# zm0612/funny_lidar_slam

Hardware: AMD Instinct MI355X
Metric: scans/sec (64-ring×1800 pts → 1e6-pt iVox map), SE(3) err vs CPU ref (higher is better)
Workload: dtype f64; 1 GPU; BASELINE configs[1]: Velodyne-64 synthetic scan (64x1800 = 115,200 pts), point-to-plane (LoamPointToPlaneIVOX semantics, YAML config_nclt.yaml) into a 1e6-pt iVox map, 1 scan per GPU per step (the same scan on every GPU); scan_points=115200, map_points=1000000, converged=True, pre_warm_matches=256

## Files before the change

### funny_lidar_slam_amd/_lib.py

```python
from __future__ import annotations

import ctypes as C
import os
import subprocess

_HERE = os.path.dirname(os.path.abspath(__file__))
LIB_PATH = os.environ.get("FLS_REG_LIB") or os.path.join(_HERE, "libfls_reg.so")
CSRC_DIR = os.path.join(_HERE, "csrc")

EXPORTED_SYMBOLS = [
    "fls_create", "fls_destroy", "fls_add_cloud_to_local_map", "fls_match", "fls_get_fitness_score",
    "fls_scan_upload", "fls_scan_upload_raw", "fls_match_resident", "fls_match_batch", "fls_map_export", "fls_map_import", "fls_map_image_bytes", "fls_map_image_export", "fls_map_image_import", "fls_get_iteration_log", "fls_get_correspondences", "fls_map_size",
    "fls_set_profiling", "fls_get_kernel_time", "fls_get_traffic_counters", "fls_get_debug_stamps", "fls_debug_fullpiv_qr6", "fls_debug_ldlt6", "fls_debug_voxel_grid", "fls_debug_voxel_grid_timed", "fls_debug_exact_sort", "fls_debug_exact_sort_marks", "fls_voxel_grid_cloud", "fls_loop_match", "fls_status_string", "fls_abi_version", "fls_abi_revision",
    "fls_device_count",
    "fls_replicas_create", "fls_replicas_refresh", "fls_replicas_match_batch", "fls_replicas_import_ms", "fls_replicas_destroy",
    "fls_features_create", "fls_features_destroy", "fls_features_project", "fls_features_extract", "fls_features_get", "fls_features_get_time",
]
HANDOFF_SYMBOLS = ["fls_preprocess_scan_device", "fls_scan_attach_preprocessed", "fls_preprocess_get_host_bytes"]
PREPROCESS_SYMBOLS = [
    "fls_preprocess_create", "fls_preprocess_destroy", "fls_preprocess_scan", "fls_preprocess_get", "fls_preprocess_get_time",
    "fls_features_project_deskew",
] + HANDOFF_SYMBOLS

FEATURES_DEVICE_SYMBOLS = ["fls_features_device_revision", "fls_features_keep_on_device", "fls_features_get_host_bytes", "fls_features_stat",
                           "fls_scan_attach_features"]
FEAT_STAT_DEVICE_GATHERS, FEAT_STAT_DEVICE_FILTERS, FEAT_STAT_FILTER_DECLINES, FEAT_STAT_LAZY_DOWNLOADS = range(4)

INGEST_SYMBOLS = ["fls_ingest_revision", "fls_ingest_default_layout", "fls_preprocess_scan_driver", "fls_features_project_driver"]

KEYFRAMES_SYMBOLS = ["fls_keyframes_revision", "fls_keyframes_create", "fls_keyframes_destroy", "fls_keyframes_add", "fls_keyframes_add_preprocessed",
                     "fls_keyframes_count", "fls_keyframes_get", "fls_keyframes_merge", "fls_keyframes_loop_match", "fls_keyframes_stat"]

LOCALMAP_SYMBOLS = ["fls_localmap_revision", "fls_localmap_create", "fls_localmap_destroy", "fls_localmap_set_global", "fls_localmap_crop",
                    "fls_localmap_split", "fls_localmap_add_tile", "fls_localmap_tiles", "fls_localmap_get_tile", "fls_localmap_load_tiles",
                    "fls_localmap_reset", "fls_localmap_get_local", "fls_add_localmap_to_local_map", "fls_localmap_stat"]

BATCH_SYMBOLS = ["fls_batch_revision", "fls_match_batch_fused", "fls_batch_stat"]

BATCH_IVOX_SYMBOLS = ["fls_batch_ivox_revision", "fls_match_batch_shared_ivox", "fls_batch_ivox_stat"]

DEBUG_LINALG_SYMBOLS = ["fls_debug_linalg_revision", "fls_debug_plane_fit_5x3", "fls_debug_svd3", "fls_debug_lu6", "fls_debug_so3", "fls_debug_wave_sum"]

DEBUG_FIT_SYMBOLS = ["fls_debug_fit_revision", "fls_debug_plane_residual", "fls_debug_line_residual", "fls_debug_icp_point_rows", "fls_debug_rank1_mfma",
                     "fls_debug_rank1_dpp", "fls_debug_rank1x3_mfma", "fls_debug_reduce_partials", "fls_debug_fanin", "fls_debug_last_system"]
DEBUG_TICKET_WORDS = 320

DEBUG_NDT_SYMBOLS = ["fls_debug_ndt_revision", "fls_debug_ndt_voxels"]

DEBUG_LOOP_SYMBOLS = ["fls_debug_loop_revision", "fls_debug_loop_ndt", "fls_debug_loop_gicp_cov", "fls_debug_loop_gicp_corr", "fls_debug_loop_gicp_fdf",
                      "fls_debug_loop_fitness"]

DEBUG_KNN_SYMBOLS = ["fls_debug_knn_revision", "fls_debug_grid_knn5", "fls_debug_grid_knn5_dual", "fls_debug_icp_knn1"]

NDT_IMAGE_SYMBOLS = ["fls_ndt_image_revision"]
NDT_IMAGE_MAGIC, NDT_IMAGE_HEADER_BYTES, NDT_IMAGE_CARRY = b"FLSNDT01", 64, 8


class NdtImageHeader(C.Structure):

    _fields_ = [("magic", C.c_char * 8), ("revision", C.c_uint32), ("carry", C.c_uint32), ("total_bytes", C.c_uint64), ("n_voxels", C.c_uint64),
                ("next_vid", C.c_int32), ("flag_first_scan", C.c_uint32), ("ndt_voxel_size_bits", C.c_uint64), ("ndt_min_points_in_voxel", C.c_int32),
                ("ndt_max_points_in_voxel", C.c_int32), ("ndt_capacity", C.c_int32), ("reserved", C.c_uint32)]


def ndt_image_layout(n: int) -> dict:
    out, o = {}, NDT_IMAGE_HEADER_BYTES
    for name, width in (("key", 8), ("num_points", 4), ("vid", 4), ("estimated", 1), ("pending", 1), ("points", NDT_IMAGE_CARRY * 24), ("mu", 24),
                        ("sigma", 72), ("info", 72)):
        out[name] = o
        o = (o + n * width + 15) & ~15
    out["total"] = o
    return out

KD_IMAGE_SYMBOLS = ["fls_kd_image_revision", "fls_replicas_match_batch_fused"]
KD_IMAGE_MAGIC, KD_IMAGE_HEADER_BYTES = b"FLSKDM01", 224


class KdImageHeader(C.Structure):

    _fields_ = [("magic", C.c_char * 8), ("revision", C.c_uint32), ("kind", C.c_uint32), ("total_bytes", C.c_uint64), ("n_maps", C.c_uint32),
                ("is_localization_mode", C.c_uint32), ("filter_size_bits", C.c_uint32 * 2), ("local_size", C.c_uint32 * 2),
                ("point_search_thres_bits", C.c_uint64), ("gate_init", C.c_uint32), ("reserved", C.c_uint32), ("gate_last_T", C.c_double * 16),
                ("n_clouds", C.c_uint64 * 2), ("n_points", C.c_uint64 * 2)]


# ... 393 lines not shown
            L.fls_debug_fanin.restype = C.c_int
            L.fls_debug_fanin.argtypes = [C.c_int, C.c_int, C.c_int, dp, u32p, u32p]
            L.fls_debug_last_system.restype = C.c_int
            L.fls_debug_last_system.argtypes = [hp, dp, dp]
        if hasattr(L, "fls_debug_ndt_revision"):
            L.fls_debug_ndt_revision.restype = C.c_int
            L.fls_debug_ndt_revision.argtypes = []
            L.fls_debug_ndt_voxels.restype = C.c_int
            L.fls_debug_ndt_voxels.argtypes = [hp, C.c_size_t, ip, ip, ip, bp, bp, dp, dp, dp, C.POINTER(C.c_size_t)]
        if hasattr(L, "fls_debug_loop_revision"):
            i64p = C.POINTER(C.c_int64)
            L.fls_debug_loop_revision.restype = C.c_int
            L.fls_debug_loop_revision.argtypes = []
            L.fls_debug_loop_ndt.restype = C.c_int
            L.fls_debug_loop_ndt.argtypes = [C.c_int, fp, C.c_int, fp, C.c_int, C.c_int, C.c_float, dp, C.c_int, dp, dp, dp, i64p, ip, ip]
            L.fls_debug_loop_gicp_cov.restype = C.c_int
            L.fls_debug_loop_gicp_cov.argtypes = [C.c_int, fp, C.c_int, C.c_int, C.c_float, C.c_double, C.c_int, dp]
            L.fls_debug_loop_gicp_corr.restype = C.c_int
            L.fls_debug_loop_gicp_corr.argtypes = [C.c_int, fp, C.c_int, fp, C.c_int, C.c_int, fp, dp, dp, dp, C.c_double, C.c_int, ip, dp]
            L.fls_debug_loop_gicp_fdf.restype = C.c_int
            L.fls_debug_loop_gicp_fdf.argtypes = [C.c_int, fp, C.c_int, fp, C.c_int, C.c_int, dp, ip, dp, C.c_int, dp]
            L.fls_debug_loop_fitness.restype = C.c_int
            L.fls_debug_loop_fitness.argtypes = [C.c_int, fp, C.c_int, fp, C.c_int, C.c_int, fp, C.c_int, dp, i64p]
        if hasattr(L, "fls_debug_knn_revision"):
            L.fls_debug_knn_revision.restype = C.c_int
            L.fls_debug_knn_revision.argtypes = []
            L.fls_debug_grid_knn5.restype = C.c_int
            L.fls_debug_grid_knn5.argtypes = [C.c_int, fp, C.c_int, fp, C.c_int, C.c_int, C.c_float, C.c_int, C.c_float, dp, C.c_int, fp, bp, fp, ip]
            L.fls_debug_grid_knn5_dual.restype = C.c_int
            L.fls_debug_grid_knn5_dual.argtypes = [C.c_int, fp, C.c_int, fp, C.c_int, C.c_float, C.c_int, C.c_float, fp, C.c_int, fp, C.c_int, C.c_float, C.c_int,
                                                   C.c_float, C.c_int, dp, C.c_int, fp, bp, fp, ip, fp, bp, fp, ip]
            L.fls_debug_icp_knn1.restype = C.c_int
            L.fls_debug_icp_knn1.argtypes = [C.c_int, fp, C.c_int, fp, C.c_int, C.c_int, C.c_float, C.c_double, dp, C.c_int, ip, bp, ip]
        if hasattr(L, "fls_ndt_image_revision"):
            L.fls_ndt_image_revision.restype = C.c_int
            L.fls_ndt_image_revision.argtypes = []
        if hasattr(L, "fls_kd_image_revision"):
            L.fls_kd_image_revision.restype = C.c_int
            L.fls_kd_image_revision.argtypes = []
            L.fls_replicas_match_batch_fused.restype = C.c_int
            L.fls_replicas_match_batch_fused.argtypes = L.fls_replicas_match_batch.argtypes
        L.fls_status_string.restype = C.c_char_p
        L.fls_status_string.argtypes = [C.c_int]
        L.fls_abi_version.restype = C.c_int
        L.fls_abi_revision.restype = C.c_int
        L.fls_device_count.restype = C.c_int
        _lib = L
    return _lib


def status_string(s: int) -> str:
    return lib().fls_status_string(int(s)).decode()


def device_count() -> int:
    return int(lib().fls_device_count())
```

### funny_lidar_slam_amd/csrc/abi_common.hpp

```cpp
#pragma once
#include <chrono>
#include "matcher_p2plane_ivox.hpp"
#include "matchers_kd.hpp"
#include "matcher_ndt.hpp"
#include "features_host.hpp"
#include "preprocess_host.hpp"
#include "loop_closure.hpp"
#include "replicas.hpp"
#include "keyframes.hpp"
#include "localmap.hpp"
#include "kernels_debug_linalg.hpp"
#include "kernels_debug_fit.hpp"
#include "../../include/fls_keyframes.h"
#include "../../include/fls_localmap.h"
#include "../../include/fls_batch.h"
#include "../../include/fls_batch_ivox.h"
#include "../../include/fls_debug_linalg.h"
#include "../../include/fls_debug_fit.h"
#include "../../include/fls_debug_ndt.h"
#include "../../include/fls_debug_loop.h"
#include "../../include/fls_debug_knn.h"
#include "../../include/fls_map_kd.h"
#include <new>
#include <type_traits>

namespace fls {

inline fls_status gfx950_device(int device_id, bool say = false) {
    int n = 0;
    hipDeviceProp_t prop;
    if (hipGetDeviceCount(&n) != hipSuccess || device_id < 0 || device_id >= n || hipGetDeviceProperties(&prop, device_id) != hipSuccess) return FLS_ERR_DEVICE;
    const char* arch = prop.gcnArchName;
    if (std::strncmp(arch, "gfx950", 6) == 0) return FLS_OK;
    if (say) std::fprintf(stderr, "[fls_reg] device %d is %s; this library is built for gfx950 only\n", device_id, arch);
    return FLS_ERR_DEVICE;
}

template <typename F>
fls_status guarded_nomem(F&& f) {
    return guarded([&]() -> fls_status {
        try {
            return f();
        } catch (const HipError& e) {
            if (e.code != hipErrorOutOfMemory) throw;
            (void)hipGetLastError();
            return FLS_ERR_NOMEM;
        }
    });
}

template <class H, class F>
fls_status on_device(H* h, F&& body) {
    return guarded([&]() -> fls_status { FLS_HIP(hipSetDevice(h->device)); return body(); });
}
// ... 63 lines not shown
```

### funny_lidar_slam_amd/csrc/abi_debug_knn.hpp

```cpp
#pragma once
#include "abi_common.hpp"

namespace {

fls_status debug_knn_device(int device_id) {
    const fls_status dev = gfx950_device(device_id);
    if (dev == FLS_OK) FLS_HIP(hipSetDevice(device_id));
    return dev;
}
inline bool debug_knn_common_ok(const float* map, int nm, const float* query, int nq, int stride, float cell, int host_grid) {
    return map && query && nm >= 0 && nq >= 0 && stride >= 3 && cell > 0.f && std::isfinite(cell) && (host_grid == 0 || host_grid == 1);
}
struct DebugKnnSide {
    LoopMatcher::DevCloud map, query;
    CellGridImage grid;
    DeviceGridBuilder builder;
    DevBuf<float4> pts;
    DevBuf<unsigned char> cnt, flag;
    DevBuf<float> kth;
    int nq = 0;
    fls_status prepare_grid(const float* m, int nm, const float* q, int n_query, int stride, float cell, int rings, bool host_grid) {
        const std::vector<PtI> mc = cloud_from(m, size_t(nm), stride), qc = cloud_from(q, size_t(n_query), stride);
        nq = n_query;
        map.upload(mc, nullptr);
// ... 2 lines not shown
        return grid.build(mc, cell, nullptr, rings, false);
    }
    void prepare_outputs() {
        pts.reserve(size_t(nq) * 5); cnt.reserve(size_t(nq)); flag.reserve(size_t(nq)); kth.reserve(size_t(nq));
        FLS_HIP(hipMemset(pts.p, 0x7b, size_t(nq) * 5 * sizeof(float4)));
        FLS_HIP(hipMemset(cnt.p, 0x7b, size_t(nq)));
        FLS_HIP(hipMemset(flag.p, 0x7b, size_t(nq)));
        FLS_HIP(hipMemset(kth.p, 0x7b, size_t(nq) * sizeof(float)));
    }
    GridKnnArgs args(float gate) { return GridKnnArgs{query.x(), query.y(), query.z(), nq, cell_dev(grid), gate, pts.p, cnt.p, kth.p, flag.p}; }
    void fetch(float* out_pts, uint8_t* out_cnt, float* out_kth, int32_t* out_has_window) {
        FLS_HIP(hipMemcpy(out_pts, pts.p, size_t(nq) * 5 * sizeof(float4), hipMemcpyDeviceToHost));
        FLS_HIP(hipMemcpy(out_cnt, cnt.p, size_t(nq), hipMemcpyDeviceToHost));
        FLS_HIP(hipMemcpy(out_kth, kth.p, size_t(nq) * sizeof(float), hipMemcpyDeviceToHost));
        *out_has_window = grid.have_window ? 1 : 0;
    }
};
inline void debug_knn_empty(int nq, float* out_pts, uint8_t* out_cnt, float* out_kth, int32_t* out_has_window) {
    const int32_t none = -1;
    for (size_t i = 0; i < size_t(nq) * 5; ++i) {
        out_pts[4 * i] = out_pts[4 * i + 1] = out_pts[4 * i + 2] = 0.f;
        std::memcpy(out_pts + 4 * i + 3, &none, sizeof(none));
    }
    for (int i = 0; i < nq; ++i) { out_cnt[i] = 0; out_kth[i] = INFINITY; }
    *out_has_window = 0;
}
inline Pose16 debug_knn_pose(const double* T16) { Pose16 T; std::memcpy(T.m, T16, sizeof(T.m)); return T; }

}

extern "C" {

int fls_debug_knn_revision(void) { return FLS_DEBUG_KNN_REVISION; }

fls_status fls_debug_grid_knn5(int device_id, const float* map, int nm, const float* query, int nq, int stride, float cell, int rings, float gate,
                               const double* T16, int host_grid, float* out_pts, uint8_t* out_cnt, float* out_kth, int32_t* out_has_window) {
    if (!debug_knn_common_ok(map, nm, query, nq, stride, cell, host_grid) || !T16 || !out_pts || !out_cnt || !out_kth || !out_has_window || (rings != 1 && rings != 2) ||
        gate != gate)
        return FLS_ERR_INVALID;
    if (nm == 0 || nq == 0) { debug_knn_empty(nq, out_pts, out_cnt, out_kth, out_has_window); return FLS_OK; }
    return guarded([&]() -> fls_status {
        fls_status rc = debug_knn_device(device_id);
        if (rc != FLS_OK) return rc;
        DebugKnnSide s;
        rc = s.prepare_grid(map, nm, query, nq, stride, cell, rings, host_grid != 0);
        if (rc != FLS_OK) return rc;
        s.prepare_outputs();
        DevBuf<GnState> st;
        st.reserve(1);
        FLS_HIP(hipMemset(st.p, 0, sizeof(GnState)));
        const GridKnnArgs a = s.args(gate);
        const dim3 knn_grid_dim(knn_grid_blocks(size_t(nq)));
        const Pose16 T0 = debug_knn_pose(T16);
        if (std::isinf(gate))
            hipLaunchKernelGGL((grid_knn_kernel<5, false, true>), knn_grid_dim, dim3(256), 0, nullptr, a.sx, a.sy, a.sz, a.n, (const GnState*)st.p, 1, T0, a.cg, gate, a.nn_pts,
                               a.nn_cnt, a.kth_d2, a.flag_to_clear);
        else
            hipLaunchKernelGGL((grid_knn_kernel<5, false>), knn_grid_dim, dim3(256), 0, nullptr, a.sx, a.sy, a.sz, a.n, (const GnState*)st.p, 1, T0, a.cg, gate, a.nn_pts,
                               a.nn_cnt, a.kth_d2, a.flag_to_clear);
        FLS_HIP(hipGetLastError());
        FLS_HIP(hipDeviceSynchronize());
        s.fetch(out_pts, out_cnt, out_kth, out_has_window);
        return FLS_OK;
    });
}

// ... 71 lines not shown
```

### funny_lidar_slam_amd/csrc/device_common.hpp

```cpp
#pragma once
#include <hip/hip_runtime.h>
#include <stdint.h>

namespace fls {

constexpr int kMaxIter = 64;
constexpr int kPartialStride = 32;
constexpr unsigned long long kEmptyKey = ~0ull;
constexpr int kKeyLimit = (1 << 20) - 2;

struct HashEntry {
    unsigned long long key;
    unsigned begin;
    unsigned count;
};
static_assert(sizeof(HashEntry) == 16, "one dwordx4 per probe");

struct DevGrid {
    const HashEntry* table;
    const float4* pts;
    unsigned mask;
    unsigned n_pts;
};

// ... 149 lines not shown
#pragma unroll
    for (int k = 0; k < NV; ++k) p[k] = a[k] = 0u;
    for (int j = threadIdx.x; j < n; j += blockDim.x) {
        const T4 e = v[j];
        const unsigned* w = reinterpret_cast<const unsigned*>(&e);
#pragma unroll
        for (int k = 0; k < NV; ++k) { a[k] += w[k]; if (j < cut) p[k] += w[k]; }
    }
    const int lane = threadIdx.x & 63, wv = threadIdx.x >> 6, nw = blockDim.x >> 6;
#pragma unroll
    for (int k = 0; k < NV; ++k) {
#pragma unroll
        for (int o = 32; o > 0; o >>= 1) { p[k] += __shfl_xor(p[k], o, 64); a[k] += __shfl_xor(a[k], o, 64); }
    }
    if (lane == 0) {
#pragma unroll
        for (int k = 0; k < NV; ++k) { wsum[wv][k] = p[k]; wsum[wv][NV + k] = a[k]; }
    }
    __syncthreads();
#pragma unroll
    for (int k = 0; k < NV; ++k) {
        unsigned sp = 0u, sa = 0u;
        for (int q = 0; q < nw; ++q) { sp += wsum[q][k]; sa += wsum[q][NV + k]; }
        pre[k] = sp; all[k] = sa;
    }
    __syncthreads();
}
#endif

struct Pose16 { double m[16]; };

struct TrafficCounters {
    unsigned long long probes, hits, cand;
};

__host__ __device__ __forceinline__ unsigned long long pack_key(int x, int y, int z) {
    return ((unsigned long long)((unsigned)x & 0x1FFFFFu) << 42) | ((unsigned long long)((unsigned)y & 0x1FFFFFu) << 21) |
           (unsigned long long)((unsigned)z & 0x1FFFFFu);
}
__host__ __device__ __forceinline__ void unpack_key(unsigned long long k, int& x, int& y, int& z) {
    x = (int)((unsigned)(k >> 42) << 11) >> 11;
    y = (int)((unsigned)((k >> 21) & 0x1FFFFFu) << 11) >> 11;
    z = (int)((unsigned)(k & 0x1FFFFFu) << 11) >> 11;
}
__host__ __device__ __forceinline__ unsigned hash_key(unsigned long long k) {
    k ^= k >> 33;
    k *= 0xff51afd7ed558ccdULL;
    k ^= k >> 33;
    k *= 0xc4ceb9fe1a85ec53ULL;
    k ^= k >> 33;
    return (unsigned)k;
}

__device__ __forceinline__ unsigned evict_merged_rank(const unsigned* __restrict__ crank, const unsigned C, const unsigned* S, const unsigned nS, const unsigned k) {
    unsigned j = 0;
    while (j < nS && j <= k && S[j] < (k - j < C ? crank[k - j] : 0xFFFFFFFFu)) ++j;
    unsigned v = 0u;
    if (j <= k && k - j < C) v = crank[k - j];
    if (j > 0u && S[j - 1] > v) v = S[j - 1];
    return v;
}

}
```

### funny_lidar_slam_amd/csrc/kernels_ivox_coop.hpp

```cpp
#pragma once
#include "kernels_p2plane.hpp"
#include "lane_group.hpp"

namespace fls {

__device__ __forceinline__ void nearby18(const int k, int& dx, int& dy, int& dz) {
    constexpr unsigned long long DX = 0x1548889561ull, DY = 0x895429495ull, DZ = 0x282956155ull;
    dx = (int)((DX >> (2 * k)) & 3ull) - 1;
    dy = (int)((DY >> (2 * k)) & 3ull) - 1;
    dz = (int)((DZ >> (2 * k)) & 3ull) - 1;
}

constexpr int nearby18_slab(const int k) {
    constexpr unsigned long long DX = 0x1548889561ull, DY = 0x895429495ull, DZ = 0x282956155ull;
    const int dx = (int)((DX >> (2 * k)) & 3ull) - 1, dy = (int)((DY >> (2 * k)) & 3ull) - 1, dz = (int)((DZ >> (2 * k)) & 3ull) - 1;
    return (dz * kBrickStored + dy) * kBrickStored + dx;
}
constexpr unsigned nearby18_slab_pack4(const int r) {
    unsigned pk = 0u;
    for (int s = 0; s < 4; ++s) {
        const int k = s + 4 * r;
        pk |= ((unsigned)(k < 19 ? nearby18_slab(k) : 0) & 0xffu) << (8 * s);
    }
    return pk;
// ... 4 lines not shown
__device__ __forceinline__ double kmin_f64(const double a, const double b) {
    double r;
    asm("v_min_f64 %0, %1, %2" : "=v"(r) : "v"(a), "v"(b));
    return r;
}
__device__ __forceinline__ double kmax_f64(const double a, const double b) {
    double r;
    asm("v_max_f64 %0, %1, %2" : "=v"(r) : "v"(a), "v"(b));
    return r;
}
__device__ __forceinline__ double make_dkey(const float d2, const unsigned slot, const bool ok) {
    return __hiloint2double((int)(ok ? __float_as_uint(d2) + kKeyBias : kKeyNoneHi), (int)slot);
}
__device__ __forceinline__ bool dkey_valid(const double k) { return (unsigned)__double2hiint(k) < kKeyValidLimit; }
__device__ __forceinline__ unsigned dkey_slot(const double k) { return (unsigned)__double2loint(k); }
__device__ __forceinline__ void top5_insert_dkey(double (&t)[5], const double key) {
    double x = kmin_f64(t[4], key);
#pragma unroll
    for (int j = 3; j >= 0; --j) {
        const double lo = kmin_f64(t[j], x), hi = kmax_f64(t[j], x);
        t[j + 1] = hi;
        x = lo;
    }
    t[0] = x;
}
template <int STEP>
__device__ __forceinline__ double dpp_min_dkey(const double v) {
    const unsigned lo = dpp_pair_u32<STEP>((unsigned)__double2loint(v));
    const unsigned hi = dpp_pair_u32<STEP>((unsigned)__double2hiint(v));
    return kmin_f64(v, __hiloint2double((int)hi, (int)lo));
}
__device__ __forceinline__ double group_min_dkey(const double v) { return dpp_min_dkey<1>(dpp_min_dkey<0>(v)); }

constexpr int kIvoxKnnQueries = 256 / 4;
#define FLS_IVOX_KNN_SMEM_PARAMS unsigned (&s_end)[kIvoxKnnQueries][24], unsigned (&s_off)[kIvoxKnnQueries][24]
#define FLS_IVOX_KNN_SMEM_DECL                                                             \
    __shared__ __attribute__((aligned(16))) unsigned s_end[kIvoxKnnQueries][24];           \
    __shared__ __attribute__((aligned(16))) unsigned s_off[kIvoxKnnQueries][24]
#define FLS_IVOX_KNN_SMEM_ARGS s_end, s_off
template <bool COUNT, bool DENSE, bool FIRST, bool GEN, class P>
__device__ __forceinline__ void
ivox_knn_body(FLS_IVOX_KNN_SMEM_PARAMS, const float* __restrict__ sx, const float* __restrict__ sy, const float* __restrict__ sz, const int n,
              const GnState* __restrict__ st, const P& T0p , const DevGrid grid, const BrickDir bd,
              const float inv_res, float4* __restrict__ nn_pts , unsigned char* __restrict__ nn_cnt,
              unsigned char* __restrict__ flag, TrafficCounters* __restrict__ tc, const int chunk,
              unsigned* __restrict__ nn_ids ,
              const int nn_prev ,
              float* __restrict__ dev_copy ) {
    const Pose16& T0 = T0p;
    constexpr int G = 4;
    constexpr int QPB = kIvoxKnnQueries;
    constexpr int R = (19 + G - 1) / G;
    const int nb = (n + QPB - 1) / QPB;
    const int xcd = blockIdx.x & 7, seq = blockIdx.x >> 3;
    const int lb = ((seq / chunk) * 8 + xcd) * chunk + (seq % chunk);
    const int sub = threadIdx.x % G;
    const int q = lb * QPB + threadIdx.x / G;
    const bool active = lb < nb && q < n;
    const int done = FIRST ? 0 : st->done;
    double T[12];
#pragma unroll
    for (int c = 0; c < 4; ++c)
#pragma unroll
        for (int r = 0; r < 3; ++r) T[c * 3 + r] = FIRST ? T0.m[c * 4 + r] : st->T[c * 4 + r];
    const int qq = active ? q : 0;
    const float px = sx[qq], py = sy[qq], pz = sz[qq];
    if (done) return;
    if (FIRST && active && sub == 0) {
        if (dev_copy) { dev_copy[q] = px; dev_copy[(size_t)n + q] = py; dev_copy[2 * (size_t)n + q] = pz; }
        flag[q] = 0;
        if (q >= nn_prev) nn_cnt[q] = 0;
    }
    const double x = px, y = py, z = pz;
    const float ptx = (float)(((T[0] * x + T[3] * y) + T[6] * z) + T[9]);
    const float pty = (float)(((T[1] * x + T[4] * y) + T[7] * z) + T[10]);
    const float ptz = (float)(((T[2] * x + T[5] * y) + T[8] * z) + T[11]);
    const float fx = roundf(ptx * inv_res), fy = roundf(pty * inv_res), fz = roundf(ptz * inv_res);
    const bool in_range = active && fabsf(fx) < (float)kKeyLimit && fabsf(fy) < (float)kKeyLimit && fabsf(fz) < (float)kKeyLimit;
    const int kx = in_range ? (int)fx : 0, ky = in_range ? (int)fy : 0, kz = in_range ? (int)fz : 0;

    const double kNone = __hiloint2double((int)kKeyNoneHi, -1);
    double t5[5] = {kNone, kNone, kNone, kNone, kNone};
    unsigned long long c_hits = 0, c_cand = 0, c_probes = 0;
    auto probe_key = [&](const int r, bool& pv) -> unsigned long long {
        const int k = sub + G * r;
        pv = in_range && k < 19;
        int ox, oy, oz;
        nearby18(k < 19 ? k : 0, ox, oy, oz);
        return pack_key(kx + ox, ky + oy, kz + oz);
    };
    auto first_load = [&](const bool pv, const unsigned long long key, unsigned& h) -> HashEntry {
        h = hash_key(key) & grid.mask;
        return pv ? grid.table[h] : HashEntry{kEmptyKey, 0u, 0u};
    };
    auto resolve = [&](const bool pv, const unsigned long long key, unsigned h, HashEntry ek, unsigned& beg, unsigned& cnt) {
        while (pv && ek.key != key && ek.key != kEmptyKey) {
            h = (h + 1) & grid.mask;
            ek = grid.table[h];
        }
        const bool hit = pv && ek.key == key;
        beg = hit ? ek.begin : 0u;
        cnt = hit ? ek.count : 0u;
        if (COUNT && pv) { c_probes++; if (hit) { c_hits++; c_cand += ek.count; } }
    };
    unsigned b0 = 0, b1 = 0, b2 = 0, b3 = 0, b4 = 0, c0 = 0, c1 = 0, c2 = 0, c3 = 0, c4 = 0;
    if (DENSE) {
        const int bx = kx >> kBrickLog, by = ky >> kBrickLog, bz = kz >> kBrickLog;
        const unsigned long long bkey = pack_key(bx, by, bz);
        unsigned h = brick_hash(bx, by, bz) & bd.mask;
        HashEntry be = bd.table[h];
        while (be.key != bkey && be.key != kEmptyKey) {
            h = (h + 1) & bd.mask;
            be = bd.table[h];
        }
        const bool have = in_range && be.key == bkey && be.begin < bd.n_cap;
        const unsigned cbase = (have ? be.begin : 0u) * kBrickStride +
                               brick_slab_index((kx & (kBrickSide - 1)) + 1, (ky & (kBrickSide - 1)) + 1, (kz & (kBrickSide - 1)) + 1);
        constexpr unsigned PK[5] = {nearby18_slab_pack4(0), nearby18_slab_pack4(1), nearby18_slab_pack4(2), nearby18_slab_pack4(3), nearby18_slab_pack4(4)};
        const unsigned sub8 = 8u * (unsigned)sub;
        auto cell = [&](const int r, const unsigned pk4, unsigned& beg, unsigned& cnt) {
            const int k = sub + G * r;
            const int off = __builtin_amdgcn_sbfe((int)pk4, sub8, 8u);
            const bool ok = have && k < 19;
            const uint2 e = bd.cells[cbase + (unsigned)off];
            beg = e.x;
            cnt = ok ? e.y : 0u;
            if (COUNT && active && k < 19) { c_probes++; if (cnt) { c_hits++; c_cand += cnt; } }
        };
        cell(0, PK[0], b0, c0);
        cell(1, PK[1], b1, c1);
        cell(2, PK[2], b2, c2);
        cell(3, PK[3], b3, c3);
        cell(4, PK[4], b4, c4);
    } else {
        bool pv0 = false, pv1 = false, pv2 = false, pv3 = false, pv4 = false;
        unsigned long long k0 = 0, k1 = 0, k2 = 0, k3 = 0, k4 = 0;
        unsigned h0 = 0, h1 = 0, h2 = 0, h3 = 0, h4 = 0;
        HashEntry e0{kEmptyKey, 0u, 0u}, e1 = e0, e2 = e0, e3 = e0, e4 = e0;
        k0 = probe_key(0, pv0); e0 = first_load(pv0, k0, h0);
        k1 = probe_key(1, pv1); e1 = first_load(pv1, k1, h1);
        k2 = probe_key(2, pv2); e2 = first_load(pv2, k2, h2);
        k3 = probe_key(3, pv3); e3 = first_load(pv3, k3, h3);
        k4 = probe_key(4, pv4); e4 = first_load(pv4, k4, h4);
        resolve(pv0, k0, h0, e0, b0, c0);
        resolve(pv1, k1, h1, e1, b1, c1);
        resolve(pv2, k2, h2, e2, b2, c2);
        resolve(pv3, k3, h3, e3, b3, c3);
        resolve(pv4, k4, h4, e4, b4, c4);
        if (COUNT && active && !in_range) {
#pragma unroll
            for (int r = 0; r < R; ++r) c_probes += sub + G * r < 19 ? 1u : 0u;
        }
    }
    auto consider = [&](const float4 p, const unsigned s, const bool ok) {
        const float dx = p.x - ptx, dy = p.y - pty, dz = p.z - ptz;
        const float d2 = dx * dx + (dy * dy + dz * dz);
        top5_insert_dkey(t5, make_dkey(d2, s, GEN ? ok && d2 < 25.0f : ok));
    };
    auto map_pt = [&](const unsigned s) -> float4 {
        if (GEN) return grid.pts[s];
        return *reinterpret_cast<const float4*>(reinterpret_cast<const char*>(grid.pts) + (s << 4));
    };
    const unsigned tot = c0 + c1 + c2 + c3 + c4;
    const int g = threadIdx.x / G;
    const unsigned nz = (c0 ? 1u : 0u) + (c1 ? 1u : 0u) + (c2 ? 1u : 0u) + (c3 ? 1u : 0u) + (c4 ? 1u : 0u);
    const unsigned packed = tot * 32u + nz;
    const unsigned t0 = (unsigned)__builtin_amdgcn_update_dpp(0, (int)packed, 0x00, 0xf, 0xf, true);
    const unsigned t1 = (unsigned)__builtin_amdgcn_update_dpp(0, (int)packed, 0x55, 0xf, 0xf, true);
    const unsigned t2 = (unsigned)__builtin_amdgcn_update_dpp(0, (int)packed, 0xAA, 0xf, 0xf, true);
    const unsigned t3 = (unsigned)__builtin_amdgcn_update_dpp(0, (int)packed, 0xFF, 0xf, 0xf, true);
    const unsigned before = (sub > 0 ? t0 : 0u) + (sub > 1 ? t1 : 0u) + (sub > 2 ? t2 : 0u), all = t0 + t1 + t2 + t3;
    const unsigned TOT = all >> 5;
    unsigned pos = before & 31u, run = before >> 5;
    {
        uint2* const rowp = reinterpret_cast<uint2*>(&s_end[g][6 * sub]);
        rowp[0] = make_uint2(~0u, ~0u); rowp[1] = make_uint2(~0u, ~0u); rowp[2] = make_uint2(~0u, ~0u);
    }
    const unsigned dmy = 20u + (unsigned)sub;
    auto put = [&](const unsigned b, const unsigned c) {
        const unsigned at = c ? pos : dmy;
        s_off[g][at] = b - run;
        run += c;
        s_end[g][at] = run;
        pos += c ? 1u : 0u;
    };
    put(b0, c0);
    put(b1, c1);
    put(b2, c2);
    put(b3, c3);
    put(b4, c4);
    s_end[g][dmy] = ~0u;
    __builtin_amdgcn_fence(__ATOMIC_RELEASE, "wavefront");
    __builtin_amdgcn_wave_barrier();
    __builtin_amdgcn_fence(__ATOMIC_ACQUIRE, "wavefront");
    const unsigned Q = (TOT + 3u) >> 2, a = sub * Q, e = a + Q < TOT ? a + Q : TOT;
    const unsigned P2 = t0 + t1, P3 = P2 + t2, A32 = a * 32u + 31u;
    unsigned ps = t0 <= A32 ? t0 : 0u;
    ps = P2 <= A32 ? P2 : ps;
    ps = P3 <= A32 ? P3 : ps;
    unsigned k = ps & 31u;
    {
        const unsigned* const w = &s_end[g][k];
        const unsigned w0 = w[0], w1 = w[1], w2 = w[2], w3 = w[3], w4 = w[4];
        k += (w0 <= a ? 1u : 0u) + (w1 <= a ? 1u : 0u) + (w2 <= a ? 1u : 0u) + (w3 <= a ? 1u : 0u) + (w4 <= a ? 1u : 0u);
    }
    for (unsigned idx = a; idx < e;) {
        const unsigned E0 = s_end[g][k], E1 = s_end[g][k + 1];
        const unsigned O0 = s_off[g][k], O1 = s_off[g][k + 1];
        const unsigned last = (E1 < e ? E1 : e) - 1;
        const unsigned i1 = idx + 1, i2 = idx + 2, i3 = idx + 3;
        const unsigned j1 = i1 < last ? i1 : last, j2 = i2 < last ? i2 : last, j3 = i3 < last ? i3 : last;
        const unsigned s0 = idx + O0;
        const unsigned s1 = j1 + (j1 < E0 ? O0 : O1);
        const unsigned s2 = j2 + (j2 < E0 ? O0 : O1);
        const unsigned s3 = j3 + (j3 < E0 ? O0 : O1);
        const float4 q0 = map_pt(s0), q1 = map_pt(s1), q2 = map_pt(s2), q3 = map_pt(s3);
        consider(q0, s0, true);
        consider(q1, s1, i1 <= last);
        consider(q2, s2, i2 <= last);
        consider(q3, s3, i3 <= last);
        idx = j3 + 1;
        k += (E0 <= idx ? 1u : 0u) + (E1 <= idx ? 1u : 0u);
    }
    const double m0 = group_min_dkey(t5[0]);
    if (dkey_valid(m0)) {
        int cnt = 0;
        unsigned sid[5] = {~0u, ~0u, ~0u, ~0u, ~0u};
#pragma unroll
        for (int j = 0; j < 5; ++j) {
            const double m = j == 0 ? m0 : group_min_dkey(t5[0]);
            const bool mv = dkey_valid(m);
            cnt += mv ? 1 : 0;
            if (mv && __double_as_longlong(t5[0]) == __double_as_longlong(m)) {
                t5[0] = t5[1]; t5[1] = t5[2]; t5[2] = t5[3]; t5[3] = t5[4]; t5[4] = kNone;
            }
            if (nn_ids) sid[j] = mv ? dkey_slot(m) : ~0u;
            else if (sub == 0 && active) {
                nn_pts[(size_t)q * 5 + j] = mv ? grid.pts[dkey_slot(m)] : make_float4(0.f, 0.f, 0.f, __int_as_float(-1));
            }
        }
        if (nn_ids) {
            if (sub == 0 && active) {
                *reinterpret_cast<uint4*>(nn_ids + (size_t)q * 8) = make_uint4(sid[0], sid[1], sid[2], sid[3]);
                nn_ids[(size_t)q * 8 + 4] = sid[4];
            }
            if (sub == 0 && active) nn_cnt[q] = (unsigned char)cnt;
        } else {
            if (sub == 0 && active) nn_cnt[q] = (unsigned char)(cnt | 0x80);
        }
    }
    if (COUNT) {
        const double p = wave_sum_u((double)c_probes), hsum = wave_sum_u((double)c_hits), c = wave_sum_u((double)c_cand);
        if ((threadIdx.x & 63) == 0) {
            atomicAdd(&tc->probes, (unsigned long long)p);
            atomicAdd(&tc->hits, (unsigned long long)hsum);
// ... 366 lines not shown
```

### funny_lidar_slam_amd/csrc/matcher_base.hpp

```cpp
#pragma once
#include "host_maps.hpp"
#include "kernels_handoff.hpp"
#include "kernels_p2plane.hpp"
#include <functional>
#include <memory>
#include <thread>
#if defined(__SSE__)
#include <xmmintrin.h>
#endif

struct fls_matcher {
    fls_kind kind;
    fls_params p{};
    int device = 0;
    hipStream_t stream = nullptr;
    fls_stats stats{};

    fls::DevBuf<fls::GnState> d_state;
    fls::PinnedBuf<fls::GnState> h_state;
    fls::DevBuf<double> d_partials_a, d_partials_b;
    fls::DevBuf<fls::TrafficCounters> d_tc;
    fls::PinnedBuf<fls::TrafficCounters> h_tc;

    bool profiling = false;
    bool count_traffic = false;
    static constexpr int kEvRing = 64;
    std::vector<hipEvent_t> ev_pool;
    hipEvent_t* ev = nullptr;
    int ev_slot = -1;
    struct PendingEv { int slot, iters; };
    std::vector<PendingEv> ev_pending;
    double prof_ms = 0.0;
    int64_t prof_launches = 0;
    uint64_t prof_point_iters = 0;
    fls::TrafficCounters last_tc{0, 0, 0};

    int log_n = 0;
    bool log_stale = false;

    fls::Mailbox* mb_host = nullptr;
    fls::Mailbox* mb_dev = nullptr;
    unsigned match_id = 0;
    bool tail_exact = false;
    unsigned launch_word() const { return fls::LaunchWord::pack(match_id, tail_exact, p.max_iterations).w; }

    virtual ~fls_matcher() {
        for (hipEvent_t e : slot_ev) if (e) (void)hipEventDestroy(e);
        for (hipEvent_t e : batch_tail_ev) if (e) (void)hipEventDestroy(e);
        if (batch_stream) { (void)hipStreamSynchronize(batch_stream); (void)hipStreamDestroy(batch_stream); }
        for (auto e : ev_pool) if (e) (void)hipEventDestroy(e);
        if (stream) { (void)hipStreamSynchronize(stream); (void)hipStreamDestroy(stream); }
        if (mb_host) (void)hipHostFree(mb_host);
    }
    virtual fls_status add_cloud(const float* c0, size_t n0, const float* c1, size_t n1, int stride) = 0;
    using HostRows = std::function<const std::vector<fls::PtI>&()>;
    virtual fls_status add_cloud_device(const fls::HandoffCloud&, const HostRows& rows, bool* took_planes) {
        *took_planes = false;
        const std::vector<fls::PtI>& r = rows();
        return add_cloud(r.empty() ? nullptr : &r[0].x, r.size(), nullptr, 0, 4);
    }
    virtual fls_status scan_upload(const float* s0, size_t n0, const float* s1, size_t n1, int stride) = 0;
    virtual fls_status scan_upload_for_match(const float* s0, size_t n0, const float* s1, size_t n1, int stride) { return scan_upload(s0, n0, s1, n1, stride); }
    virtual fls_status scan_upload_raw(const float* s0, size_t n0, const float* s1, size_t n1, int stride) { return scan_upload(s0, n0, s1, n1, stride); }
    virtual fls_status scan_attach_device(const fls::HandoffCloud&) { return FLS_ERR_STATE; }
    virtual fls_status scan_attach_features(const fls::HandoffCloud& , const fls::HandoffCloud& ) { return FLS_ERR_STATE; }
    virtual fls_status match_resident(double* T, int update_map, fls_stats* out) = 0;
    virtual fls_status fitness(float max_range, float* score) = 0;
    virtual int correspondences(int slot, int32_t* ids, uint8_t* cnt, uint8_t* valid, size_t cap) = 0;
// ... 435 lines not shown
```

### funny_lidar_slam_amd/csrc/matcher_p2plane_ivox.hpp

```cpp
#pragma once
#include "matcher_base.hpp"
#include "kernels_p2plane.hpp"
#include "kernels_knn.hpp"
#include "kernels_ivox_coop.hpp"
#include "kernels_ivox_update.hpp"
#include "ivox_map.hpp"
#include "kernels_localmap.hpp"
#include "fitness_host.hpp"
#include <thread>
#include <chrono>
#include <hip/hip_ext.h>

namespace fls {

constexpr int kIvoxXcdChunk = 8;

struct P2PlaneIvoxMatcher final : fls_matcher {
    IvoxMap map;
    const IvoxMap* borrowed = nullptr;
    const IvoxMap& read_map() const { return borrowed ? *borrowed : map; }
    bool host_timing = false;
    bool spec_pending = false;
    DevBuf<unsigned char> d_code;
    DevBuf<float4> d_pw;
// ... 523 lines not shown

    std::unique_ptr<fls_matcher> clone_for_lane() override {
        auto q = make_lane(*this);
        if (q) q->borrowed = &map;
        return q;
    }
    fls_status prepare_batch() override {
        map.refresh();
        FLS_HIP(hipStreamSynchronize(stream));
        return FLS_OK;
    }

    fls_status fitness(float max_range, float* score) override {
        if (!p.is_localization_mode) { *score = std::numeric_limits<float>::max(); return FLS_OK; }
        if (!have_fitness_grid || !have_final) return FLS_ERR_STATE;
        return fitness_score_device(*this, fitness_grid, scan, final_T, max_range, score);
    }

    int correspondences(int, int32_t* ids, uint8_t* cnt, uint8_t* valid, size_t cap) override {
        download_nn();
        const size_t n = std::min(cap, nn_n);
        h_flag.resize(nn_n);
        if (nn_n) {
            FLS_HIP(hipMemcpyAsync(h_flag.data(), d_flag.p, nn_n, hipMemcpyDeviceToHost, stream));
            FLS_HIP(hipStreamSynchronize(stream));
        }
        for (size_t i = 0; i < n; ++i) {
            cnt[i] = h_cnt[i];
            for (int j = 0; j < 5; ++j) ids[i * 5 + j] = j < h_cnt[i] ? h_nn[i * 5 + j].id : -1;
            valid[i] = h_flag[i];
        }
        return int(n);
    }
    size_t map_size(int slot) const override { return map.counter(slot); }
};

}
```

### funny_lidar_slam_amd/registration.py

```python
from __future__ import annotations

import ctypes as C
from dataclasses import dataclass, field

import numpy as np

from . import _lib
from ._lib import FlsError, Params, Stats

FloatNaN = float(np.finfo(np.float32).max)

kPointToPlane_IVOX_HIP = "PointToPlane_IVOX_HIP"
kPointToPlane_KdTree_HIP = "PointToPlane_KdTree_HIP"
kLoamFull_KdTree_HIP = "LoamFull_KdTree_HIP"
kIcpOptimized_HIP = "IcpOptimized_HIP"
kIncrementalNDT_HIP = "IncrementalNDT_HIP"


@dataclass
class PointcloudCluster:
    ordered_cloud_: np.ndarray = field(default_factory=lambda: np.zeros((0, 3), np.float32))
    planar_cloud_: np.ndarray = field(default_factory=lambda: np.zeros((0, 3), np.float32))
    corner_cloud_: np.ndarray = field(default_factory=lambda: np.zeros((0, 3), np.float32))
    raw_cloud_: np.ndarray = None
# ... 241 lines not shown
    def map_size(self, slot: int = 0) -> int:
        return int(_lib.lib().fls_map_size(self._h, slot))

    def ndt_voxels(self) -> dict:
        L = _lib.lib()
        cnt = C.c_size_t(0)
        rc = L.fls_debug_ndt_voxels(self._h, 0, None, None, None, None, None, None, None, None, C.byref(cnt))
        if rc not in (_lib.FLS_OK, _lib.FLS_ERR_NOMEM):
            raise FlsError(rc, "fls_debug_ndt_voxels")
        n = int(cnt.value)
        out = dict(keys=np.zeros((n, 3), np.int32), vid=np.zeros(n, np.int32), num_points=np.zeros(n, np.int32), estimated=np.zeros(n, np.uint8),
                   pending=np.zeros(n, np.uint8), mu=np.zeros((n, 3)), sigma=np.zeros((n, 9)), info=np.zeros((n, 9)))
        if n:
            ip, bp, dp = C.POINTER(C.c_int32), C.POINTER(C.c_uint8), C.POINTER(C.c_double)
            rc = L.fls_debug_ndt_voxels(self._h, n, out["keys"].ctypes.data_as(ip), out["vid"].ctypes.data_as(ip), out["num_points"].ctypes.data_as(ip),
                                        out["estimated"].ctypes.data_as(bp), out["pending"].ctypes.data_as(bp), out["mu"].ctypes.data_as(dp),
                                        out["sigma"].ctypes.data_as(dp), out["info"].ctypes.data_as(dp), C.byref(cnt))
            if rc != _lib.FLS_OK or int(cnt.value) != n:
                raise FlsError(rc, "fls_debug_ndt_voxels")
        return out

    def set_profiling(self, events: bool, counters: bool = False) -> None:
        _lib.lib().fls_set_profiling(self._h, (1 if events else 0) | (2 if counters else 0))

    def kernel_time(self):
        ms = C.c_double(); n = C.c_int64(); pi = C.c_uint64()
        _lib.lib().fls_get_kernel_time(self._h, C.byref(ms), C.byref(n), C.byref(pi))
        return ms.value, n.value, pi.value

    def traffic_counters(self):
        a = C.c_uint64(); b = C.c_uint64(); c = C.c_uint64()
        _lib.lib().fls_get_traffic_counters(self._h, C.byref(a), C.byref(b), C.byref(c))
        return a.value, b.value, c.value

    def close(self) -> None:
        if getattr(self, "_h", None) and self._h.value:
            _lib.lib().fls_destroy(self._h)
            self._h = C.c_void_p()

    def __del__(self):
        try:
            self.close()
        except Exception:
            pass


class LoamPointToPlaneIVOX(RegistrationInterface):

    KIND = _lib.P2PLANE_IVOX

    def __init__(self, point_to_planar_thres, position_converge_thres, rotation_converge_thres, opti_iter_num=30,
                 is_localization_mode=False, device_id=0):
        super().__init__(Params(point_to_planar_thres=point_to_planar_thres, position_converge_thres=position_converge_thres,
                                rotation_converge_thres=rotation_converge_thres, max_iterations=opti_iter_num,
                                is_localization_mode=int(is_localization_mode)), device_id)


class IcpOptimized(RegistrationInterface):

    KIND = _lib.ICP_OPTIMIZED
    K = 1

    def __init__(self, max_iterations, local_map_size, map_cloud_filter_size, source_cloud_filter_size, max_correspond_distance,
                 position_converge_thres, rotation_converge_thres, rot_thre_add_cloud, dist_thre_add_cloud,
                 is_localization_mode=False, device_id=0):
        super().__init__(Params(max_iterations=max_iterations, local_map_size=local_map_size,
# ... 189 lines not shown
```

Before: 11170 scans/s.

## Share iVox KNN candidate staging across queries in the same voxel within a wave

Adds a wave-level shared path to the dense iVox KNN. When the wave's 16 queries fall into at most three distinct voxels and their combined 19-cell neighbourhoods hold at most 256 candidates, the wave probes the cells once and stages the map points in LDS. Each query group then scans its run's staged candidates instead of probing and gathering independently. This is meant to cut redundant hash probes and global point loads for spatially coherent scans. In exchange it adds ballot, scan and barrier overhead, and it falls back to the old path when the run or capacity limits are exceeded.

```diff
diff --git a/funny_lidar_slam_amd/_lib.py b/funny_lidar_slam_amd/_lib.py
--- a/funny_lidar_slam_amd/_lib.py
+++ b/funny_lidar_slam_amd/_lib.py
@@ -51,6 +51,8 @@
                       "fls_debug_loop_fitness"]
 
 DEBUG_KNN_SYMBOLS = ["fls_debug_knn_revision", "fls_debug_grid_knn5", "fls_debug_grid_knn5_dual", "fls_debug_icp_knn1"]
+
+DEBUG_IVOX_KNN_SYMBOLS = ["fls_debug_ivox_knn_revision", "fls_debug_ivox_knn_limits"]
 
 NDT_IMAGE_SYMBOLS = ["fls_ndt_image_revision"]
 NDT_IMAGE_MAGIC, NDT_IMAGE_HEADER_BYTES, NDT_IMAGE_CARRY = b"FLSNDT01", 64, 8
@@ -510,6 +512,11 @@
                                                    C.c_float, C.c_int, dp, C.c_int, fp, bp, fp, ip, fp, bp, fp, ip]
             L.fls_debug_icp_knn1.restype = C.c_int
             L.fls_debug_icp_knn1.argtypes = [C.c_int, fp, C.c_int, fp, C.c_int, C.c_int, C.c_float, C.c_double, dp, C.c_int, ip, bp, ip]
+        if hasattr(L, "fls_debug_ivox_knn_revision"):
+            L.fls_debug_ivox_knn_revision.restype = C.c_int
+            L.fls_debug_ivox_knn_revision.argtypes = []
+            L.fls_debug_ivox_knn_limits.restype = C.c_int
+            L.fls_debug_ivox_knn_limits.argtypes = [C.POINTER(C.c_int), C.POINTER(C.c_int)]
         if hasattr(L, "fls_ndt_image_revision"):
             L.fls_ndt_image_revision.restype = C.c_int
             L.fls_ndt_image_revision.argtypes = []
diff --git a/funny_lidar_slam_amd/csrc/abi_common.hpp b/funny_lidar_slam_amd/csrc/abi_common.hpp
--- a/funny_lidar_slam_amd/csrc/abi_common.hpp
+++ b/funny_lidar_slam_amd/csrc/abi_common.hpp
@@ -20,6 +20,7 @@
 #include "../../include/fls_debug_ndt.h"
 #include "../../include/fls_debug_loop.h"
 #include "../../include/fls_debug_knn.h"
+#include "../../include/fls_debug_ivox_knn.h"
 #include "../../include/fls_map_kd.h"
 #include <new>
 #include <type_traits>
diff --git a/funny_lidar_slam_amd/csrc/abi_debug_knn.hpp b/funny_lidar_slam_amd/csrc/abi_debug_knn.hpp
--- a/funny_lidar_slam_amd/csrc/abi_debug_knn.hpp
+++ b/funny_lidar_slam_amd/csrc/abi_debug_knn.hpp
@@ -58,6 +58,14 @@
 extern "C" {
 
 int fls_debug_knn_revision(void) { return FLS_DEBUG_KNN_REVISION; }
+
+int fls_debug_ivox_knn_revision(void) { return FLS_DEBUG_IVOX_KNN_REVISION; }
+fls_status fls_debug_ivox_knn_limits(int* r_max, int* cap) {
+    if (!r_max || !cap) return FLS_ERR_INVALID;
+    *r_max = kIvoxKnnRunMax;
+    *cap = kIvoxKnnStageCap;
+    return FLS_OK;
+}
 
 fls_status fls_debug_grid_knn5(int device_id, const float* map, int nm, const float* query, int nq, int stride, float cell, int rings, float gate,
                                const double* T16, int host_grid, float* out_pts, uint8_t* out_cnt, float* out_kth, int32_t* out_has_window) {
diff --git a/funny_lidar_slam_amd/csrc/device_common.hpp b/funny_lidar_slam_amd/csrc/device_common.hpp
--- a/funny_lidar_slam_amd/csrc/device_common.hpp
+++ b/funny_lidar_slam_amd/csrc/device_common.hpp
@@ -205,6 +205,7 @@
 
 struct TrafficCounters {
     unsigned long long probes, hits, cand;
+    unsigned long long shared;
 };
 
 __host__ __device__ __forceinline__ unsigned long long pack_key(int x, int y, int z) {
diff --git a/funny_lidar_slam_amd/csrc/kernels_ivox_coop.hpp b/funny_lidar_slam_amd/csrc/kernels_ivox_coop.hpp
--- a/funny_lidar_slam_amd/csrc/kernels_ivox_coop.hpp
+++ b/funny_lidar_slam_amd/csrc/kernels_ivox_coop.hpp
@@ -60,12 +60,17 @@
 }
 __device__ __forceinline__ double group_min_dkey(const double v) { return dpp_min_dkey<1>(dpp_min_dkey<0>(v)); }
 
+constexpr int kIvoxKnnRunMax = 3;
+constexpr int kIvoxKnnStageCap = 256;
 constexpr int kIvoxKnnQueries = 256 / 4;
-#define FLS_IVOX_KNN_SMEM_PARAMS unsigned (&s_end)[kIvoxKnnQueries][24], unsigned (&s_off)[kIvoxKnnQueries][24]
-#define FLS_IVOX_KNN_SMEM_DECL                                                             \
-    __shared__ __attribute__((aligned(16))) unsigned s_end[kIvoxKnnQueries][24];           \
-    __shared__ __attribute__((aligned(16))) unsigned s_off[kIvoxKnnQueries][24]
-#define FLS_IVOX_KNN_SMEM_ARGS s_end, s_off
+constexpr int kIvoxKnnWaveWords = kIvoxKnnStageCap * 4;
+static_assert(kIvoxKnnWaveWords >= 2 * 16 * 24, "the per-query tables of a wave fit its region");
+static_assert(4 * kIvoxKnnWaveWords * sizeof(unsigned) <= 20480, "eight workgroups per CU: the 1,800-workgroup launch stays one round");
+static_assert(kIvoxKnnRunMax * 19 <= 64 && kIvoxKnnStageCap <= 4 * 64, "one probe pass, four staged rows per lane");
+static_assert(kIvoxKnnRunMax == 3, "the leader and range selects of the shared path are written out for three runs");
+#define FLS_IVOX_KNN_SMEM_PARAMS unsigned (&s_knn)[256 / 64][kIvoxKnnWaveWords]
+#define FLS_IVOX_KNN_SMEM_DECL __shared__ __attribute__((aligned(16))) unsigned s_knn[256 / 64][kIvoxKnnWaveWords]
+#define FLS_IVOX_KNN_SMEM_ARGS s_knn
 template <bool COUNT, bool DENSE, bool FIRST, bool GEN, class P>
 __device__ __forceinline__ void
 ivox_knn_body(FLS_IVOX_KNN_SMEM_PARAMS, const float* __restrict__ sx, const float* __restrict__ sy, const float* __restrict__ sz, const int n,
@@ -84,6 +89,9 @@
     const int lb = ((seq / chunk) * 8 + xcd) * chunk + (seq % chunk);
     const int sub = threadIdx.x % G;
     const int q = lb * QPB + threadIdx.x / G;
+    unsigned* const s_wave = &s_knn[threadIdx.x >> 6][0];
+    unsigned* const s_end = s_wave + 24 * ((threadIdx.x / G) & 15);
+    unsigned* const s_off = s_end + 16 * 24;
     const bool active = lb < nb && q < n;
     const int done = FIRST ? 0 : st->done;
     double T[12];
@@ -131,7 +139,17 @@
         cnt = hit ? ek.count : 0u;
         if (COUNT && pv) { c_probes++; if (hit) { c_hits++; c_cand += ek.count; } }
     };
-    unsigned b0 = 0, b1 = 0, b2 = 0, b3 = 0, b4 = 0, c0 = 0, c1 = 0, c2 = 0, c3 = 0, c4 = 0;
+    auto consider = [&](const float4 p, const unsigned s, const bool ok) {
+        const float dx = p.x - ptx, dy = p.y - pty, dz = p.z - ptz;
+        const float d2 = dx * dx + (dy * dy + dz * dz);
+        top5_insert_dkey(t5, make_dkey(d2, s, GEN ? ok && d2 < 25.0f : ok));
+    };
+    auto map_pt = [&](const unsigned s) -> float4 {
+        if (GEN) return grid.pts[s];
+        return *reinterpret_cast<const float4*>(reinterpret_cast<const char*>(grid.pts) + (s << 4));
+    };
+    bool have = false;
+    unsigned cbase = 0u;
     if (DENSE) {
         const int bx = kx >> kBrickLog, by = ky >> kBrickLog, bz = kz >> kBrickLog;
         const unsigned long long bkey = pack_key(bx, by, bz);
@@ -141,9 +159,90 @@
             h = (h + 1) & bd.mask;
             be = bd.table[h];
         }
-        const bool have = in_range && be.key == bkey && be.begin < bd.n_cap;
-        const unsigned cbase = (have ? be.begin : 0u) * kBrickStride +
-                               brick_slab_index((kx & (kBrickSide - 1)) + 1, (ky & (kBrickSide - 1)) + 1, (kz & (kBrickSide - 1)) + 1);
+        have = in_range && be.key == bkey && be.begin < bd.n_cap;
+        cbase = (have ? be.begin : 0u) * kBrickStride +
+                brick_slab_index((kx & (kBrickSide - 1)) + 1, (ky & (kBrickSide - 1)) + 1, (kz & (kBrickSide - 1)) + 1);
+    }
+    bool shared = false;
+    if (DENSE && !GEN) {
+        const unsigned lane = threadIdx.x & 63u;
+        const int kxh = kx * 2 + (have ? 1 : 0);
+        const int pkx = __shfl_up(kxh, G, 64), pky = __shfl_up(ky, G, 64), pkz = __shfl_up(kz, G, 64);
+        const bool start = lane < (unsigned)G || pkx != kxh || pky != ky || pkz != kz;
+        const unsigned long long starts = __ballot(start) & 0x1111111111111111ull;
+        const int nruns = __popcll(starts);
+        if (nruns <= kIvoxKnnRunMax) {
+            const unsigned long long rest1 = starts & (starts - 1ull), rest2 = rest1 & (rest1 - 1ull), have_mask = __ballot(have);
+            const int l1 = rest1 ? __ffsll((long long)rest1) - 1 : 0, l2 = rest2 ? __ffsll((long long)rest2) - 1 : 0;
+            const unsigned cb0 = (unsigned)__builtin_amdgcn_readlane((int)cbase, 0), cb1 = (unsigned)__builtin_amdgcn_readlane((int)cbase, l1),
+                           cb2 = (unsigned)__builtin_amdgcn_readlane((int)cbase, l2);
+            const bool hv0 = (have_mask & 1ull) != 0ull, hv1 = rest1 != 0ull && ((have_mask >> l1) & 1ull) != 0ull,
+                       hv2 = rest2 != 0ull && ((have_mask >> l2) & 1ull) != 0ull;
+            const unsigned pr = lane / 19u, pk = lane - 19u * pr;
+            int ox, oy, oz;
+            nearby18((int)pk, ox, oy, oz);
+            const int poff = (oz * kBrickStored + oy) * kBrickStored + ox;
+            const unsigned pcb = pr == 0u ? cb0 : pr == 1u ? cb1 : cb2;
+            const bool phv = pr == 0u ? hv0 : pr == 1u ? hv1 : pr == 2u ? hv2 : false;
+            const uint2 pe = bd.cells[pcb + (unsigned)poff];
+            const unsigned pbeg = pe.x, pcnt_all = phv ? pe.y : 0u;
+            const unsigned pcnt = pcnt_all < (unsigned)kIvoxKnnStageCap + 1u ? pcnt_all : (unsigned)kIvoxKnnStageCap + 1u;
+            unsigned inc = pcnt;
+#pragma unroll
+            for (int o = 1; o < 64; o <<= 1) {
+                const unsigned t = __shfl_up(inc, o, 64);
+                if (lane >= (unsigned)o) inc += t;
+            }
+            const unsigned pex = inc - pcnt;
+            const unsigned total = (unsigned)__builtin_amdgcn_readlane((int)inc, 63);
+            if (total <= (unsigned)kIvoxKnnStageCap) {
+                shared = true;
+                const unsigned S1 = (unsigned)__builtin_amdgcn_readlane((int)pex, 19), S2 = (unsigned)__builtin_amdgcn_readlane((int)pex, 38);
+                const int my_run = __popcll(starts & ((2ull << lane) - 1ull)) - 1;
+                const unsigned sh_beg = my_run == 0 ? 0u : my_run == 1 ? S1 : S2, sh_end = my_run == 0 ? S1 : my_run == 1 ? S2 : total;
+                if (COUNT) {
+                    const unsigned long long hit_mask = __ballot(pcnt != 0u);
+                    const unsigned hits_run = (unsigned)__popcll((hit_mask >> (19 * my_run)) & 0x7FFFFull);
+                    if (active && sub == 0) { c_probes += 19u; c_hits += hits_run; c_cand += sh_end - sh_beg; }
+                    if (__ballot(active) != 0ull && lane == 0u) atomicAdd(&tc->shared, 1ull);
+                }
+                for (unsigned i = 0u; i < pcnt; ++i) s_wave[4u * (pex + i) + 3u] = pbeg + i;
+                __builtin_amdgcn_fence(__ATOMIC_RELEASE, "wavefront");
+                __builtin_amdgcn_wave_barrier();
+                __builtin_amdgcn_fence(__ATOMIC_ACQUIRE, "wavefront");
+                uint4* const stage = reinterpret_cast<uint4*>(s_wave);
+                unsigned sl[4] = {0u, 0u, 0u, 0u};
+                float4 sp[4];
+#pragma unroll
+                for (int j = 0; j < 4; ++j) {
+                    const unsigned en = lane + 64u * (unsigned)j;
+                    sp[j] = make_float4(0.f, 0.f, 0.f, 0.f);
+                    if (en < total) { sl[j] = s_wave[4u * en + 3u]; sp[j] = map_pt(sl[j]); }
+                }
+#pragma unroll
+                for (int j = 0; j < 4; ++j) {
+                    const unsigned en = lane + 64u * (unsigned)j;
+                    if (en < total) stage[en] = make_uint4(__float_as_uint(sp[j].x), __float_as_uint(sp[j].y), __float_as_uint(sp[j].z), sl[j]);
+                }
+                __builtin_amdgcn_fence(__ATOMIC_RELEASE, "wavefront");
+                __builtin_amdgcn_wave_barrier();
+                __builtin_amdgcn_fence(__ATOMIC_ACQUIRE, "wavefront");
+                const unsigned C = sh_end - sh_beg, Q = (C + 3u) >> 2, a = (unsigned)sub * Q, e = a + Q < C ? a + Q : C;
+                const uint4* const runp = stage + sh_beg;
+                for (unsigned idx = a; idx < e; idx += 4u) {
+                    const unsigned last = e - 1u, i1 = idx + 1u, i2 = idx + 2u, i3 = idx + 3u;
+                    const uint4 r0 = runp[idx], r1 = runp[i1 < last ? i1 : last], r2 = runp[i2 < last ? i2 : last], r3 = runp[i3 < last ? i3 : last];
+                    consider(make_float4(__uint_as_float(r0.x), __uint_as_float(r0.y), __uint_as_float(r0.z), 0.f), r0.w, true);
+                    consider(make_float4(__uint_as_float(r1.x), __uint_as_float(r1.y), __uint_as_float(r1.z), 0.f), r1.w, i1 <= last);
+                    consider(make_float4(__uint_as_float(r2.x), __uint_as_float(r2.y), __uint_as_float(r2.z), 0.f), r2.w, i2 <= last);
+                    consider(make_float4(__uint_as_float(r3.x), __uint_as_float(r3.y), __uint_as_float(r3.z), 0.f), r3.w, i3 <= last);
+                }
+            }
+        }
+    }
+    unsigned b0 = 0, b1 = 0, b2 = 0, b3 = 0, b4 = 0, c0 = 0, c1 = 0, c2 = 0, c3 = 0, c4 = 0;
+    if (shared) {
+    } else if (DENSE) {
         constexpr unsigned PK[5] = {nearby18_slab_pack4(0), nearby18_slab_pack4(1), nearby18_slab_pack4(2), nearby18_slab_pack4(3), nearby18_slab_pack4(4)};
         const unsigned sub8 = 8u * (unsigned)sub;
         auto cell = [&](const int r, const unsigned pk4, unsigned& beg, unsigned& cnt) {
@@ -180,17 +279,8 @@
             for (int r = 0; r < R; ++r) c_probes += sub + G * r < 19 ? 1u : 0u;
         }
     }
-    auto consider = [&](const float4 p, const unsigned s, const bool ok) {
-        const float dx = p.x - ptx, dy = p.y - pty, dz = p.z - ptz;
-        const float d2 = dx * dx + (dy * dy + dz * dz);
-        top5_insert_dkey(t5, make_dkey(d2, s, GEN ? ok && d2 < 25.0f : ok));
-    };
-    auto map_pt = [&](const unsigned s) -> float4 {
-        if (GEN) return grid.pts[s];
-        return *reinterpret_cast<const float4*>(reinterpret_cast<const char*>(grid.pts) + (s << 4));
-    };
+    if (!shared) {
     const unsigned tot = c0 + c1 + c2 + c3 + c4;
-    const int g = threadIdx.x / G;
     const unsigned nz = (c0 ? 1u : 0u) + (c1 ? 1u : 0u) + (c2 ? 1u : 0u) + (c3 ? 1u : 0u) + (c4 ? 1u : 0u);
     const unsigned packed = tot * 32u + nz;
     const unsigned t0 = (unsigned)__builtin_amdgcn_update_dpp(0, (int)packed, 0x00, 0xf, 0xf, true);
@@ -201,15 +291,15 @@
     const unsigned TOT = all >> 5;
     unsigned pos = before & 31u, run = before >> 5;
     {
-        uint2* const rowp = reinterpret_cast<uint2*>(&s_end[g][6 * sub]);
+        uint2* const rowp = reinterpret_cast<uint2*>(&s_end[6 * sub]);
         rowp[0] = make_uint2(~0u, ~0u); rowp[1] = make_uint2(~0u, ~0u); rowp[2] = make_uint2(~0u, ~0u);
     }
     const unsigned dmy = 20u + (unsigned)sub;
     auto put = [&](const unsigned b, const unsigned c) {
         const unsigned at = c ? pos : dmy;
-        s_off[g][at] = b - run;
+        s_off[at] = b - run;
         run += c;
-        s_end[g][at] = run;
+        s_end[at] = run;
         pos += c ? 1u : 0u;
     };
     put(b0, c0);
@@ -217,7 +307,7 @@
     put(b2, c2);
     put(b3, c3);
     put(b4, c4);
-    s_end[g][dmy] = ~0u;
+    s_end[dmy] = ~0u;
     __builtin_amdgcn_fence(__ATOMIC_RELEASE, "wavefront");
     __builtin_amdgcn_wave_barrier();
     __builtin_amdgcn_fence(__ATOMIC_ACQUIRE, "wavefront");
@@ -228,13 +318,13 @@
     ps = P3 <= A32 ? P3 : ps;
     unsigned k = ps & 31u;
     {
-        const unsigned* const w = &s_end[g][k];
+        const unsigned* const w = &s_end[k];
         const unsigned w0 = w[0], w1 = w[1], w2 = w[2], w3 = w[3], w4 = w[4];
         k += (w0 <= a ? 1u : 0u) + (w1 <= a ? 1u : 0u) + (w2 <= a ? 1u : 0u) + (w3 <= a ? 1u : 0u) + (w4 <= a ? 1u : 0u);
     }
     for (unsigned idx = a; idx < e;) {
-        const unsigned E0 = s_end[g][k], E1 = s_end[g][k + 1];
-        const unsigned O0 = s_off[g][k], O1 = s_off[g][k + 1];
+        const unsigned E0 = s_end[k], E1 = s_end[k + 1];
+        const unsigned O0 = s_off[k], O1 = s_off[k + 1];
         const unsigned last = (E1 < e ? E1 : e) - 1;
         const unsigned i1 = idx + 1, i2 = idx + 2, i3 = idx + 3;
         const unsigned j1 = i1 < last ? i1 : last, j2 = i2 < last ? i2 : last, j3 = i3 < last ? i3 : last;
@@ -249,6 +339,7 @@
         consider(q3, s3, i3 <= last);
         idx = j3 + 1;
         k += (E0 <= idx ? 1u : 0u) + (E1 <= idx ? 1u : 0u);
+    }
     }
     const double m0 = group_min_dkey(t5[0]);
     if (dkey_valid(m0)) {
diff --git a/funny_lidar_slam_amd/csrc/matcher_base.hpp b/funny_lidar_slam_amd/csrc/matcher_base.hpp
--- a/funny_lidar_slam_amd/csrc/matcher_base.hpp
+++ b/funny_lidar_slam_amd/csrc/matcher_base.hpp
@@ -33,7 +33,7 @@
     double prof_ms = 0.0;
     int64_t prof_launches = 0;
     uint64_t prof_point_iters = 0;
-    fls::TrafficCounters last_tc{0, 0, 0};
+    fls::TrafficCounters last_tc{0, 0, 0, 0};
 
     int log_n = 0;
     bool log_stale = false;
diff --git a/funny_lidar_slam_amd/csrc/matcher_p2plane_ivox.hpp b/funny_lidar_slam_amd/csrc/matcher_p2plane_ivox.hpp
--- a/funny_lidar_slam_amd/csrc/matcher_p2plane_ivox.hpp
+++ b/funny_lidar_slam_amd/csrc/matcher_p2plane_ivox.hpp
@@ -579,7 +579,7 @@
         }
         return int(n);
     }
-    size_t map_size(int slot) const override { return map.counter(slot); }
+    size_t map_size(int slot) const override { return slot == 176 ? size_t(last_tc.shared) : map.counter(slot); }
 };
 
 }
diff --git a/funny_lidar_slam_amd/registration.py b/funny_lidar_slam_amd/registration.py
--- a/funny_lidar_slam_amd/registration.py
+++ b/funny_lidar_slam_amd/registration.py
@@ -297,6 +297,9 @@
         a = C.c_uint64(); b = C.c_uint64(); c = C.c_uint64()
         _lib.lib().fls_get_traffic_counters(self._h, C.byref(a), C.byref(b), C.byref(c))
         return a.value, b.value, c.value
+
+    def knn_shared_waves(self) -> int:
+        return self.map_size(176)
 
     def close(self) -> None:
         if getattr(self, "_h", None) and self._h.value:
diff --git a/include/fls_debug_ivox_knn.h b/include/fls_debug_ivox_knn.h
--- /dev/null
+++ b/include/fls_debug_ivox_knn.h
@@ -0,0 +1,17 @@
+#ifndef FLS_DEBUG_IVOX_KNN_H
+#define FLS_DEBUG_IVOX_KNN_H
+#include "fls_reg.h"
+#ifdef __cplusplus
+extern "C" {
+#endif
+
+#define FLS_DEBUG_IVOX_KNN_REVISION 1
+
+int fls_debug_ivox_knn_revision(void);
+
+fls_status fls_debug_ivox_knn_limits(int* r_max, int* cap);
+
+#ifdef __cplusplus
+}
+#endif
+#endif
```

After: 11400 scans/s (median of 6 runs). No clear change (+2.1%).
